# pranoyr/attention-models

Measured on AMD Instinct MI355X. Metric: ViTVQGAN 256px train-step images/sec, higher is better.
Workload: dtype f32; 1 GPU; BASELINE.json configs[2]: ViTVQGAN dim=256 patch=8 img=256 depth=6+6 h=8 d=64 mlp=2048 (SwiGLU), codebook 8192x32; GAN train step (D phase + G phase, gradient penalty, per_loss_weight=0), Adam, clip 1.0; global_batch=32, batch_per_gpu=32, parallelism=dp1

## Files before the change

attention-models_amd/amk/lib.py:

```python
import ctypes
import os
import re

_HERE = os.path.dirname(os.path.abspath(__file__))
LIB_PATH = os.environ.get("AMK_LIB") or os.path.join(_HERE, "libamk.so")
HEADER_PATH = os.path.normpath(os.path.join(_HERE, "..", "..", "include", "amk.h"))

AMK_OK = 0

_c = ctypes
_P = _c.c_void_p
_I = _c.c_int
_L = _c.c_int64
_F = _c.c_float



class GemmDesc(_c.Structure):
    _fields_ = [("op", _c.c_int32), ("epilogue", _c.c_int32), ("m", _L),
                ("n", _c.c_int32), ("k", _c.c_int32), ("split", _c.c_int32), ("reserved", _c.c_int32),
                ("a", _P), ("a2", _P), ("w", _P), ("w2", _P), ("c", _P), ("c2", _P),
                ("lda", _L), ("lda2", _L), ("ldw", _L), ("ldw2", _L), ("ldc", _L), ("ldc2", _L),
                ("bias", _P), ("bias2", _P), ("resid", _P), ("ldr", _L),
                ("ln_mean", _P), ("ln_rstd", _P), ("ln_gamma", _P), ("ln_beta", _P),
                ("ab", _P), ("ldab", _L), ("gate", _P), ("ldg", _L), ("dbias", _P)]


GEMM_NT, GEMM_NN, GEMM_TN = 0, 1, 2
EPI_BIAS, EPI_RESID, EPI_SWIGLU, EPI_SWIGLU_BWD = 0, 1, 2, 3

SIGNATURES = {
    "amk_version": (_I, []),
    "amk_arch": (_c.c_char_p, []),
    "amk_last_error": (_c.c_char_p, []),
    "amk_attn_fwd": (_I, [_P] * 7 + [_I] * 5 + [_L] * 12 + [_F, _P]),
    "amk_attn_scores_bytes": (_L, [_I, _I, _I, _I]),
    "amk_attn_fwd_keep": (_I, [_P] * 8 + [_I] * 5 + [_L] * 12 + [_F, _P]),
    "amk_attn_fwd_x6_ws_bytes": (_L, [_I, _I, _I]),
    "amk_attn_fwd_x6": (_I, [_P] * 8 + [_I] * 5 + [_L] * 12 + [_F, _P]),
    "amk_attn_bwd_ws_floats": (_L, [_I, _I, _I, _I, _I]),
    "amk_attn_bwd": (_I, [_P] * 12 + [_I] * 5 + [_L] * 24 + [_F, _I, _P]),
    "amk_attn_bwd_kept": (_I, [_P] * 13 + [_I] * 5 + [_L] * 24 + [_F, _I, _P]),
    "amk_vq_num_partials": (_L, [_L]),
    "amk_vq_lookup_fwd": (_I, [_P, _P, _L, _I, _I, _I] + [_P] * 9 + [_P]),
    "amk_vq_lookup_bwd": (_I, [_P] * 7 + [_F, _L, _I, _I, _P, _P, _P]),
    "amk_vq_lookup_bwd_rows": (_I, [_P] * 7 + [_F, _L, _I, _I, _P, _P, _P]),
    "amk_vq_padded_codes": (_I, [_I, _I]),
    "amk_vq_gather": (_I, [_P, _P, _L, _I, _I, _P, _P, _P]),
    "amk_agent_num_chunks": (_I, [_I]),
    "amk_agent_ws_floats": (_L, [_I, _I, _I, _I, _I]),
    "amk_agent_num_chunks_dh": (_I, [_I, _I]),
    "amk_agent_ws_floats_dh": (_L, [_I, _I, _I, _I, _I, _I]),
    "amk_agent_attn_fwd": (_I, [_P] * 10 + [_I] * 5 + [_L] * 12 + [_F, _P]),
    "amk_agent_attn_bwd": (_I, [_P] * 14 + [_I] * 5 + [_L] * 21 + [_F, _P]),
    "amk_agent_conv_grad_reduce": (_I, [_P, _P, _L, _I, _P, _P, _P]),
    "amk_rowsum_num_partials": (_I, [_L]),
    "amk_add_layernorm_fwd": (_I, [_P, _P, _P, _P, _L, _I, _F, _P, _P, _P, _P, _P]),
    "amk_add_layernorm_bwd": (_I, [_P, _P, _P, _P, _P, _P, _L, _I, _P, _P, _P]),
    "amk_colsum": (_I, [_P, _L, _I, _P, _P]),
    "amk_swiglu_fwd": (_I, [_P, _L, _I, _P, _P]),
    "amk_swiglu_bwd": (_I, [_P, _P, _L, _I, _P, _P]),
    "amk_geglu_fwd": (_I, [_P, _L, _I, _P, _P]),
# ... 89 lines not shown
```

attention-models_amd/amk/ops.py:

```python
import ctypes
import os
import weakref

import torch
from torch.autograd.function import once_differentiable

from . import lib as _lib

_NULL = ctypes.c_void_p(0)


def _ptr(t):
    return ctypes.c_void_p(t.data_ptr()) if t is not None else _NULL


def _stream():
    return ctypes.c_void_p(torch.cuda.current_stream().cuda_stream)


KERNEL_EVENTS = None


class _timed:

# ... 49 lines not shown
def _as_kernel_view(t):
    if _kernel_view_ok(t):
        return t
    B, H, T, D = t.shape
    return t.permute(0, 2, 1, 3).contiguous().permute(0, 2, 1, 3)


def _new_bthd(B, H, T, D, like):
    return torch.empty((B, T, H, D), device=like.device, dtype=torch.float32).permute(0, 2, 1, 3)


def _mask_u8(mask, shape, what):
    if mask is None:
        return None
    m = mask
    while m.dim() > len(shape) and m.shape[0] == 1:
        m = m[0]
    if m.dim() != len(shape):
        raise RuntimeError(f"{what} must have {len(shape)} dims (got shape {tuple(mask.shape)})")
    m = m.expand(*shape)
    return m.to(torch.uint8).contiguous()


ATTENTION_FORWARD = os.environ.get("AMK_ATTENTION_FORWARD", "f32")

ATTENTION_KEEP_SCORES = os.environ.get("AMK_ATTN_KEEP_SCORES", "1") == "1"
ATTENTION_KEEP_SCORES_MAX_BYTES = 8 << 30
ATTENTION_KEEP_SCORES_BUDGET_BYTES = int(os.environ.get("AMK_ATTN_KEEP_BUDGET", "0")) or None
_kept_scores_bytes = [0]


def _keep_budget(device):
    if ATTENTION_KEEP_SCORES_BUDGET_BYTES is not None:
        return ATTENTION_KEEP_SCORES_BUDGET_BYTES
    return torch.cuda.get_device_properties(device).total_memory // 4


def _release_kept(nbytes):
    _kept_scores_bytes[0] -= nbytes
ATTENTION_BACKWARD_KEYS = int(os.environ.get("AMK_ATTN_BWD_KEYS", "0"))


def _attn_forward(q, k, v, key_mask, causal_mask, scale, keep_scores=False):
    B, H, I, D = q.shape
    J = k.shape[2]
    _require_device(q, k, v, key_mask, causal_mask)
    if k.shape != (B, H, J, D) or v.shape != (B, H, J, D):
        raise RuntimeError(f"attention shapes disagree: q {tuple(q.shape)} k {tuple(k.shape)} v {tuple(v.shape)}")
    q, k, v = _as_kernel_view(q), _as_kernel_view(k), _as_kernel_view(v)
    o = _new_bthd(B, H, I, D, q)
    stats = torch.empty((B, H, I, 2), device=q.device, dtype=torch.float32)
    L = _lib.load()
    x6 = ATTENTION_FORWARD == "bf16x6" and D == 64
    ws = torch.empty((L.amk_attn_fwd_x6_ws_bytes(B, H, J),), device=q.device, dtype=torch.uint8) if x6 else None
    scores = None
    det = DETERMINISTIC_ATTENTION_BACKWARD or torch.are_deterministic_algorithms_enabled()
    keepable = D == 64 or (D == 128 and key_mask is None and causal_mask is None and not det)
    if (keep_scores and keepable and not x6 and ATTENTION_KEEP_SCORES
            and not ATTENTION_BACKWARD_TWO_KERNEL):
        nbytes = L.amk_attn_scores_bytes(B, H, I, J)
        if nbytes <= ATTENTION_KEEP_SCORES_MAX_BYTES and _kept_scores_bytes[0] + nbytes <= _keep_budget(q.device):
            scores = torch.empty((nbytes // 4,), device=q.device, dtype=torch.float32)
            _kept_scores_bytes[0] += nbytes
            weakref.finalize(scores.untyped_storage(), _release_kept, nbytes)
    with _timed("attn_fwd_keep_kernel" if scores is not None else "attn_fwd_kernel"):
        if scores is not None:
            rc = L.amk_attn_fwd_keep(
                _ptr(q), _ptr(k), _ptr(v), _ptr(o), _ptr(stats), _ptr(scores), _ptr(key_mask), _ptr(causal_mask),
                B, H, I, J, D, *_strides4(q), *_strides4(k), *_strides4(v), *_strides4(o),
                float(scale), _stream(),
            )
        elif x6:
            rc = L.amk_attn_fwd_x6(
                _ptr(q), _ptr(k), _ptr(v), _ptr(o), _ptr(stats), _ptr(ws), _ptr(key_mask), _ptr(causal_mask),
                B, H, I, J, D, *_strides4(q), *_strides4(k), *_strides4(v), *_strides4(o),
                float(scale), _stream(),
            )
        else:
            rc = L.amk_attn_fwd(
                _ptr(q), _ptr(k), _ptr(v), _ptr(o), _ptr(stats), _ptr(key_mask), _ptr(causal_mask),
                B, H, I, J, D, *_strides4(q), *_strides4(k), *_strides4(v), *_strides4(o),
                float(scale), _stream(),
            )
    _lib.check(rc, "amk_attn_fwd")
    return q, k, v, o, stats, scores


DETERMINISTIC_ATTENTION_BACKWARD = os.environ.get("AMK_DETERMINISTIC", "0") == "1"
ATTENTION_BACKWARD_TWO_KERNEL = False
# ... 42 lines not shown
        )
        _lib.check(rc, "amk_attn_bwd")

    if KERNEL_EVENTS is not None and (stages & ATTN_BWD_DELTA) and (stages & ~ATTN_BWD_DELTA):
        call(ATTN_BWD_DELTA)
        name = "attn_bwd_dkdv+dq" if not stages & ATTN_BWD_FUSED else (
            "attn_bwd_fused_kernel(kept scores)" if scores is not None else "attn_bwd_fused_kernel")
        with _timed(name):
            call(stages & ~ATTN_BWD_DELTA)
    else:
        call(stages)


_amp_fwd = torch.amp.custom_fwd(device_type="cuda", cast_inputs=torch.float32)
_amp_bwd = torch.amp.custom_bwd(device_type="cuda")


class _AttnCore(torch.autograd.Function):

    @staticmethod
    @_amp_fwd
    def forward(ctx, q, k, v, key_mask, causal_mask, scale):
        need = any(ctx.needs_input_grad[:3])
        q, k, v, o, stats, scores = _attn_forward(q, k, v, key_mask, causal_mask, scale, keep_scores=need)
        ctx.save_for_backward(q, k, v, o, stats, key_mask, causal_mask, scores)
        ctx.scale = scale
        return o

    @staticmethod
    @once_differentiable
    @_amp_bwd
    def backward(ctx, d_o):
        q, k, v, o, stats, key_mask, causal_mask, scores = ctx.saved_tensors
        B, H, I, D = q.shape
        J = k.shape[2]
        dq = _new_bthd(B, H, I, D, q)
        dk = _new_bthd(B, H, J, D, q)
        dv = _new_bthd(B, H, J, D, q)
        _attn_backward(q, k, v, o, stats, d_o, dq, dk, dv, key_mask, causal_mask, ctx.scale, scores=scores)
        return dq, dk, dv, None, None, None


class _AttnFusedKV(torch.autograd.Function):

    @staticmethod
    @_amp_fwd
    def forward(ctx, q2, kv2, key_mask, causal_mask, H, D, scale):
        B, I, _ = q2.shape
        J = kv2.shape[1]
        q2 = q2.contiguous()
        kv2 = kv2.contiguous()
        q = q2.view(B, I, H, D).permute(0, 2, 1, 3)
        kv = kv2.view(B, J, 2, H, D)
        k = kv[:, :, 0].permute(0, 2, 1, 3)
        v = kv[:, :, 1].permute(0, 2, 1, 3)
        need = any(ctx.needs_input_grad[:2])
        q, k, v, o, stats, scores = _attn_forward(q, k, v, key_mask, causal_mask, scale, keep_scores=need)
        ctx.save_for_backward(q, k, v, o, stats, key_mask, causal_mask, scores)
        ctx.scale = scale
        return o.permute(0, 2, 1, 3).reshape(B, I, H * D)

    @staticmethod
    @once_differentiable
    @_amp_bwd
    def backward(ctx, d_o2):
        q, k, v, o, stats, key_mask, causal_mask, scores = ctx.saved_tensors
        B, H, I, D = q.shape
        J = k.shape[2]
        d_o = d_o2.contiguous().view(B, I, H, D).permute(0, 2, 1, 3)
        dq2 = torch.empty((B, I, H * D), device=q.device, dtype=torch.float32)
        dkv2 = torch.empty((B, J, 2 * H * D), device=q.device, dtype=torch.float32)
        dq = dq2.view(B, I, H, D).permute(0, 2, 1, 3)
        dkv = dkv2.view(B, J, 2, H, D)
        dk = dkv[:, :, 0].permute(0, 2, 1, 3)
        dv = dkv[:, :, 1].permute(0, 2, 1, 3)
        _attn_backward(q, k, v, o, stats, d_o, dq, dk, dv, key_mask, causal_mask, ctx.scale, scores=scores)
        return dq2, dkv2, None, None, None, None, None


ATTENTION_BF16 = os.environ.get("AMK_ATTENTION_BF16", "1") == "1"
# ... 1502 lines not shown
```

attention-models_amd/csrc/attn_common.h:

```cpp
#pragma once
#include "amk_common.h"

namespace amk_attn {

constexpr int D = 64;
constexpr int NWAVE = 4;
constexpr int WG = NWAVE * AMK_WAVE;
constexpr int BLK = 32 * NWAVE;
constexpr int TILE = 64;
constexpr int LDS_STRIDE = 68;

#define AMK_FILL_MASKED (-1.0e9f * AMK_LOG2E)

struct Strides {
  int64_t sb, st, sh;
};

struct FwdParams {
  const float *q, *k, *v;
  float *o, *stats;
  const uint8_t *key_mask, *causal_mask;
  int B, H, I, J;
  Strides qs, ks, vs, os;
  float scale;
// ... 51 lines not shown
#pragma unroll
    for (int ps = 0; ps < NP; ++ps) {
      dst[ps] = __builtin_bit_cast(float4, __builtin_amdgcn_raw_buffer_load_b128(rsrc, voff[ps], 0, 0));
      voff[ps] += step;
    }
  }
  __device__ __forceinline__ void seek(int blk, int64_t row_stride, int tid) {
    const int srow = tid >> 4, scol = (tid & 15) * 4;
#pragma unroll
    for (int ps = 0; ps < NP; ++ps) voff[ps] = (int)(((int64_t)(srow + RP * ps) * row_stride + scol) * 4) + blk * step;
  }
};
typedef RowStagerT<TILE> RowStager;

inline bool aligned16(const void* p) { return (reinterpret_cast<uintptr_t>(p) & 15) == 0; }
inline bool strides_ok(const Strides& s) { return (s.sb % 4 == 0) && (s.st % 4 == 0) && (s.sh % 4 == 0); }

__device__ __forceinline__ float4 ld4(const float* p) { return *reinterpret_cast<const float4*>(p); }
__device__ __forceinline__ void st4(float* p, float4 v) { *reinterpret_cast<float4*>(p) = v; }
__device__ __forceinline__ float f4(const float4& v, int e) {
  return e == 0 ? v.x : (e == 1 ? v.y : (e == 2 ? v.z : v.w));
}

void launch_attn_fwd_x6(const FwdParams& p, int64_t nwg, hipStream_t st);

bool launch_attn_bwd_fused(const BwdParams& p, int keys_per_wg, hipStream_t st);
int fused_keys_per_wg(int J, int keys_per_wg);

bool attn_gen_supported(int Dh);
void launch_attn_fwd_gen(const FwdParams& p, int Dh, int64_t nwg, hipStream_t st);
void launch_attn_bwd_gen(const BwdParams& p, int Dh, int stages, hipStream_t st);
bool launch_attn_bwd_fused_gen(const BwdParams& p, int Dh, hipStream_t st);

}
```

attention-models_amd/csrc/attn_fwd.hip:

```cpp
#include "attn_common.h"
#include <stdlib.h>
#include <type_traits>

#ifndef AMK_FWD_ABL
#define AMK_FWD_ABL 0
#endif

namespace amk_attn {

template <bool CAUSAL, bool SCHED, bool KEEP>
__global__ __launch_bounds__(WG, 2) void attn_fwd_kernel(FwdParams p) {
  __shared__ __attribute__((aligned(16))) float smem[2 * TILE * LDS_STRIDE + TILE];
  float* Ks = smem;
  float* Vs = smem + TILE * LDS_STRIDE;
  float* Kfill = smem + 2 * TILE * LDS_STRIDE;

  const int tid = threadIdx.x;
  const int lane = tid & 63, wave = tid >> 6;
  const int ln = lane & 31, hf = lane >> 5;

  const int wg = __builtin_amdgcn_readfirstlane(xcd_remap(blockIdx.x, gridDim.x));
  const int qb = __builtin_amdgcn_readfirstlane(wg % p.nblk);
  const int bh = __builtin_amdgcn_readfirstlane(wg / p.nblk);
  const int h = __builtin_amdgcn_readfirstlane(bh % p.H), b = __builtin_amdgcn_readfirstlane(bh / p.H);
// ... 457 lines not shown
  FwdParams p;
  p.q = q; p.k = k; p.v = v; p.o = o; p.stats = stats;
  p.key_mask = key_mask; p.causal_mask = causal_mask;
  p.B = B; p.H = H; p.I = I; p.J = J;
  p.qs = {q_sb, q_st, q_sh}; p.ks = {k_sb, k_st, k_sh}; p.vs = {v_sb, v_st, v_sh}; p.os = {o_sb, o_st, o_sh};
  p.scale = scale;
  p.pinf = INFINITY;
  p.nblk = (I + BLK - 1) / BLK;
  p.x6_ws = x6_ws;
  p.scores = scores;
  AMK_CHECK_ARG(!scores || aligned16(scores), "amk_attn_fwd_keep: the scores buffer must be 16-byte aligned");
  AMK_CHECK_ARG(!x6 || (x6_ws && aligned16(x6_ws)), "amk_attn_fwd_x6: workspace missing or not 16-byte aligned");
  AMK_CHECK_ARG(aligned16(q) && aligned16(k) && aligned16(v) && aligned16(o) && strides_ok(p.qs) &&
                    strides_ok(p.ks) && strides_ok(p.vs) && strides_ok(p.os),
                "amk_attn_fwd: pointers must be 16-byte aligned and strides multiples of 4 elements");
  const int64_t nwg = (int64_t)B * H * p.nblk;
  AMK_CHECK_SUPPORTED(nwg < (1ll << 31), "amk_attn_fwd: grid too large");
  AMK_CHECK_SUPPORTED(((int64_t)J + TILE) * k_st * 4 < (1ll << 31) && ((int64_t)J + TILE) * v_st * 4 < (1ll << 31),
                      "amk_attn_fwd: one (batch, head) K/V slab must span < 2 GiB");
  hipStream_t st = static_cast<hipStream_t>(stream);
  if (Dh != D)
    launch_attn_fwd_gen(p, Dh, nwg, st);
  else if (x6)
    launch_attn_fwd_x6(p, nwg, st);
  else if (!causal_mask && !key_mask && getenv_plain() && scores)
    hipLaunchKernelGGL((attn_fwd_plain_kernel<true>), dim3((unsigned)nwg), dim3(WG), 0, st, p);
  else if (!causal_mask && !key_mask && getenv_plain())
    hipLaunchKernelGGL((attn_fwd_plain_kernel<false>), dim3((unsigned)nwg), dim3(WG), 0, st, p);
  else if (causal_mask && scores)
    hipLaunchKernelGGL((attn_fwd_kernel<true, false, true>), dim3((unsigned)nwg), dim3(WG), 0, st, p);
  else if (causal_mask)
    hipLaunchKernelGGL((attn_fwd_kernel<true, false, false>), dim3((unsigned)nwg), dim3(WG), 0, st, p);
  else if (scores)
    hipLaunchKernelGGL((attn_fwd_kernel<false, true, true>), dim3((unsigned)nwg), dim3(WG), 0, st, p);
  else
    hipLaunchKernelGGL((attn_fwd_kernel<false, true, false>), dim3((unsigned)nwg), dim3(WG), 0, st, p);
  AMK_CHECK_LAUNCH("amk_attn_fwd");
  return AMK_OK;
}

extern "C" int amk_attn_fwd(const float* q, const float* k, const float* v, float* o, float* stats,
                            const uint8_t* key_mask, const uint8_t* causal_mask,
                            int B, int H, int I, int J, int Dh,
                            int64_t q_sb, int64_t q_st, int64_t q_sh,
                            int64_t k_sb, int64_t k_st, int64_t k_sh,
                            int64_t v_sb, int64_t v_st, int64_t v_sh,
                            int64_t o_sb, int64_t o_st, int64_t o_sh,
// ... 16 lines not shown
                                 int64_t o_sb, int64_t o_st, int64_t o_sh,
                                 float scale, void* stream) {
  AMK_CHECK_ARG(scores, "amk_attn_fwd_keep: null scores buffer");
  return attn_fwd_impl(nullptr, false, scores, q, k, v, o, stats, key_mask, causal_mask, B, H, I, J, Dh, q_sb, q_st, q_sh, k_sb,
                       k_st, k_sh, v_sb, v_st, v_sh, o_sb, o_st, o_sh, scale, stream);
}

extern "C" int64_t amk_attn_fwd_x6_ws_bytes(int B, int H, int J) {
  if (B <= 0 || H <= 0 || J <= 0) return 0;
  return (int64_t)B * H * ((J + TILE - 1) / TILE) * 2 * 24576;
}

extern "C" int amk_attn_fwd_x6(const float* q, const float* k, const float* v, float* o, float* stats, void* ws,
                               const uint8_t* key_mask, const uint8_t* causal_mask,
                               int B, int H, int I, int J, int Dh,
                               int64_t q_sb, int64_t q_st, int64_t q_sh,
                               int64_t k_sb, int64_t k_st, int64_t k_sh,
                               int64_t v_sb, int64_t v_st, int64_t v_sh,
                               int64_t o_sb, int64_t o_st, int64_t o_sh,
                               float scale, void* stream) {
  return attn_fwd_impl(ws, true, nullptr, q, k, v, o, stats, key_mask, causal_mask, B, H, I, J, Dh, q_sb, q_st, q_sh, k_sb, k_st, k_sh,
                       v_sb, v_st, v_sh, o_sb, o_st, o_sh, scale, stream);
}
```

attention-models_amd/csrc/attn_fwd_x6.hip:

```cpp
#include "attn_common.h"

namespace amk_attn {

typedef __bf16 bf16x8 __attribute__((ext_vector_type(8)));
typedef __bf16 bf16x4 __attribute__((ext_vector_type(4)));

constexpr int PSTR = 72;
constexpr int PLANE = TILE * PSTR;

__device__ __forceinline__ f32x16 mfmab(bf16x8 a, bf16x8 b, f32x16 c) {
  return __builtin_amdgcn_mfma_f32_32x32x16_bf16(a, b, c, 0, 0, 0);
}
__device__ __forceinline__ f32x16 mfma6(const bf16x8 (&a)[3], const bf16x8 (&b)[3], f32x16 c) {
  c = mfmab(a[1], b[1], c);
  c = mfmab(a[2], b[0], c);
  c = mfmab(a[0], b[2], c);
  c = mfmab(a[1], b[0], c);
  c = mfmab(a[0], b[1], c);
  c = mfmab(a[0], b[0], c);
  return c;
}
__device__ __forceinline__ void mfma6x2(const bf16x8 (&a0)[3], const bf16x8 (&a1)[3], const bf16x8 (&b)[3], f32x16& c0, f32x16& c1) {
  c0 = mfmab(a0[1], b[1], c0); c1 = mfmab(a1[1], b[1], c1);
  c0 = mfmab(a0[2], b[0], c0); c1 = mfmab(a1[2], b[0], c1);
// ... 6 lines not shown
  h = (__bf16)x;
  const float r1 = x - (float)h;
  m = (__bf16)r1;
  l = (__bf16)(r1 - (float)m);
}
__device__ __forceinline__ void split8(const float (&x)[8], bf16x8 (&pl)[3]) {
#pragma unroll
  for (int j = 0; j < 8; ++j) {
    __bf16 h, m, l;
    split1(x[j], h, m, l);
    pl[0][j] = h; pl[1][j] = m; pl[2][j] = l;
  }
}
__device__ __forceinline__ void split4(float a, float b, float c, float d, bf16x4 (&pl)[3]) {
  const float x[4] = {a, b, c, d};
#pragma unroll
  for (int j = 0; j < 4; ++j) {
    __bf16 h, m, l;
    split1(x[j], h, m, l);
    pl[0][j] = h; pl[1][j] = m; pl[2][j] = l;
  }
}

template <bool CAUSAL>
__global__ __launch_bounds__(WG, 2) void attn_fwd_x6_kernel(FwdParams p) {
  __shared__ __attribute__((aligned(16))) __bf16 Kp[3 * PLANE];
  __shared__ __attribute__((aligned(16))) __bf16 Vt[3 * PLANE];
  __shared__ __attribute__((aligned(16))) float Kfill[TILE];

  const int tid = threadIdx.x;
  const int lane = tid & 63, wave = tid >> 6;
  const int ln = lane & 31, hf = lane >> 5;

  const int wg = xcd_remap(blockIdx.x, gridDim.x);
  const int qb = wg % p.nblk;
  const int bh = wg / p.nblk;
  const int h = bh % p.H, b = bh / p.H;

  const int qi = qb * BLK + wave * 32 + ln;
  const bool qvalid = qi < p.I;

  bf16x8 qpl[4][3];
  {
    const float qscale = p.scale * AMK_LOG2E;
    const float* qp = p.q + (int64_t)b * p.qs.sb + (int64_t)qi * p.qs.st + (int64_t)h * p.qs.sh + 8 * hf;
#pragma unroll
    for (int c = 0; c < 4; ++c) {
      const float4 t0 = qvalid ? ld4(qp + 16 * c) : make_float4(0.f, 0.f, 0.f, 0.f);
      const float4 t1 = qvalid ? ld4(qp + 16 * c + 4) : make_float4(0.f, 0.f, 0.f, 0.f);
      const float x[8] = {t0.x * qscale, t0.y * qscale, t0.z * qscale, t0.w * qscale,
                          t1.x * qscale, t1.y * qscale, t1.z * qscale, t1.w * qscale};
      split8(x, qpl[c]);
    }
  }

  const uint8_t* kmask = p.key_mask ? p.key_mask + (int64_t)b * p.J : nullptr;
  const uint8_t* cmrow = CAUSAL ? p.causal_mask + (int64_t)qi * p.J : nullptr;

  const int ntile = (p.J + TILE - 1) / TILE;
  const __amdgpu_buffer_rsrc_t wsrc = __builtin_amdgcn_make_buffer_rsrc(
      reinterpret_cast<char*>(p.x6_ws) + (int64_t)bh * ntile * 2 * 24576, 0, ntile * 2 * 24576, 0x00020000);
  float4 kch[6], vch[6];
  int lds_off[6];
#pragma unroll
  for (int n = 0; n < 6; ++n) {
    const int c = tid + 256 * n;
    const int row = c / 24, plane = (c % 24) >> 3, k8 = c & 7;
    lds_off[n] = plane * PLANE + row * PSTR + 8 * k8;
  }
  float fillst = 0.f;
  auto prefetch = [&](int t) {
    const int base = t * 2 * 24576 + tid * 16;
#pragma unroll
    for (int n = 0; n < 6; ++n) {
      kch[n] = __builtin_bit_cast(float4, __builtin_amdgcn_raw_buffer_load_b128(wsrc, base + 4096 * n, 0, 0));
      vch[n] = __builtin_bit_cast(float4, __builtin_amdgcn_raw_buffer_load_b128(wsrc, base + 24576 + 4096 * n, 0, 0));
    }
    if (tid < TILE) {
      const int j = t * TILE + tid;
      float f = 0.f;
      if (j >= p.J) f = -INFINITY;
      else if (kmask && kmask[j] == 0) f = AMK_FILL_MASKED;
      fillst = f;
    }
  };
  auto commit = [&]() {
#pragma unroll
    for (int n = 0; n < 6; ++n) {
      *reinterpret_cast<float4*>(&Kp[lds_off[n]]) = kch[n];
      *reinterpret_cast<float4*>(&Vt[lds_off[n]]) = vch[n];
    }
    if (tid < TILE) Kfill[tid] = fillst;
  };

  f32x16 o0 = zero16(), o1 = zero16();
  float m_run = -INFINITY, l_run = 0.f;

  prefetch(0);
  for (int t = 0; t < ntile; ++t) {
    const int j0 = t * TILE;
    __syncthreads();
    commit();
    __syncthreads();
    if (t + 1 < ntile) prefetch(t + 1);

    unsigned cbits0 = 0, cbits1 = 0;
    if (CAUSAL) {
      if (qvalid) {
#pragma unroll
        for (int r = 0; r < 16; ++r) {
          const int ja = j0 + acc_row(r, hf), jb = ja + 32;
          if (ja < p.J && cmrow[ja]) cbits0 |= 1u << r;
          if (jb < p.J && cmrow[jb]) cbits1 |= 1u << r;
        }
      }
    }

    f32x16 s0 = zero16(), s1 = zero16();
#pragma unroll
    for (int c = 0; c < 4; ++c) {
      bf16x8 ka[3], kb2[3];
#pragma unroll
      for (int q = 0; q < 3; ++q) {
        ka[q] = *reinterpret_cast<const bf16x8*>(&Kp[q * PLANE + ln * PSTR + 16 * c + 8 * hf]);
        kb2[q] = *reinterpret_cast<const bf16x8*>(&Kp[q * PLANE + (32 + ln) * PSTR + 16 * c + 8 * hf]);
      }
      mfma6x2(ka, kb2, qpl[c], s0, s1);
    }

    const bool plain = !CAUSAL && kmask == nullptr && (j0 + TILE <= p.J);
    float mx;
    if (plain) {
      mx = vmax(s0[0], s1[0], p.pinf);
#pragma unroll
      for (int r = 1; r < 16; ++r) mx = vmax(mx, vmax(s0[r], s1[r], p.pinf), p.pinf);
    } else {
      mx = -INFINITY;
#pragma unroll
      for (int g = 0; g < 4; ++g) {
        const float4 f0 = ld4(&Kfill[8 * g + 4 * hf]);
        const float4 f1 = ld4(&Kfill[32 + 8 * g + 4 * hf]);
#pragma unroll
        for (int e = 0; e < 4; ++e) {
          const int r = 4 * g + e;
          float t0 = s0[r], t1 = s1[r];
          const float fa = f4(f0, e), fb = f4(f1, e);
          t0 = (fa == 0.f) ? t0 : fa;
          t1 = (fb == 0.f) ? t1 : fb;
          if (CAUSAL) {
            t0 = ((cbits0 >> r) & 1u) ? AMK_FILL_MASKED : t0;
            t1 = ((cbits1 >> r) & 1u) ? AMK_FILL_MASKED : t1;
// ... 8 lines not shown
    const float m_new = vmax(m_run, mx, p.pinf);
    f32x2 lsum2 = {0.f, 0.f};
#pragma unroll
    for (int r = 0; r < 16; ++r) {
      const float p0 = __builtin_amdgcn_exp2f(s0[r] - m_new);
      const float p1 = __builtin_amdgcn_exp2f(s1[r] - m_new);
      s0[r] = p0;
      s1[r] = p1;
      lsum2 += (f32x2){p0, p1};
    }
    const float lsum = lsum2.x + lsum2.y;
    if (__any(m_new != m_run)) {
      const float alpha = __builtin_amdgcn_exp2f(m_run - m_new);
      l_run *= alpha;
#pragma unroll
      for (int r = 0; r < 16; ++r) {
        o0[r] *= alpha;
        o1[r] *= alpha;
      }
      m_run = m_new;
    }
    l_run += lsum;

#pragma unroll
    for (int g = 0; g < 4; ++g) {
      float x[8];
#pragma unroll
      for (int j = 0; j < 8; ++j) x[j] = (g < 2) ? s0[8 * (g & 1) + j] : s1[8 * (g & 1) + j];
      bf16x8 pp[3];
      split8(x, pp);
      bf16x8 va[3], vb[3];
#pragma unroll
      for (int q = 0; q < 3; ++q) {
        va[q] = *reinterpret_cast<const bf16x8*>(&Vt[q * PLANE + ln * PSTR + 16 * g + 8 * hf]);
        vb[q] = *reinterpret_cast<const bf16x8*>(&Vt[q * PLANE + (32 + ln) * PSTR + 16 * g + 8 * hf]);
      }
      mfma6x2(va, vb, pp, o0, o1);
    }
  }

  const float l_tot = l_run + __shfl_xor(l_run, 32, 64);
  const float inv = 1.f / l_tot;
  if (qvalid) {
    float* op = p.o + (int64_t)b * p.os.sb + (int64_t)qi * p.os.st + (int64_t)h * p.os.sh + 4 * hf;
#pragma unroll
    for (int g = 0; g < 4; ++g) {
      st4(op + 8 * g, make_float4(o0[4 * g] * inv, o0[4 * g + 1] * inv, o0[4 * g + 2] * inv, o0[4 * g + 3] * inv));
      st4(op + 32 + 8 * g, make_float4(o1[4 * g] * inv, o1[4 * g + 1] * inv, o1[4 * g + 2] * inv, o1[4 * g + 3] * inv));
    }
    if (hf == 0) {
      float* sp = p.stats + (((int64_t)b * p.H + h) * p.I + qi) * 2;
      sp[0] = m_run;
      sp[1] = l_tot;
    }
  }
}

__global__ __launch_bounds__(WG) void attn_split_kv_kernel(FwdParams p) {
  const int tid = threadIdx.x;
  const int ntile = (p.J + TILE - 1) / TILE;
  const int t = blockIdx.x % ntile;
  const int bh = blockIdx.x / ntile;
  const int h = bh % p.H, b = bh / p.H;
  const float* kbase = p.k + (int64_t)b * p.ks.sb + (int64_t)h * p.ks.sh;
  const float* vbase = p.v + (int64_t)b * p.vs.sb + (int64_t)h * p.vs.sh;
  __bf16* out = reinterpret_cast<__bf16*>(p.x6_ws) + ((int64_t)bh * ntile + t) * 2 * 1536 * 8;
  const int srow = tid >> 4, scol = (tid & 15) * 4;
  RowStager kload, vload;
  kload.init(kbase, p.ks.st, p.J, tid);
  vload.init(vbase, p.vs.st, p.J, tid);
  kload.seek(t, p.ks.st, tid);
  vload.seek(t, p.vs.st, tid);
#pragma unroll
  for (int i = 0; i < 4; ++i) vload.voff[i] = (int)(((int64_t)(4 * srow + i) * p.vs.st + scol) * 4) + t * vload.step;
  float4 kst[4], vst[4];
  kload.load(kst);
  vload.load(vst);
#pragma unroll
  for (int ps = 0; ps < 4; ++ps) {
    bf16x4 pl[3];
    split4(kst[ps].x, kst[ps].y, kst[ps].z, kst[ps].w, pl);
    const int r = srow + 16 * ps;
#pragma unroll
    for (int q = 0; q < 3; ++q) *reinterpret_cast<bf16x4*>(out + (r * 3 + q) * 64 + scol) = pl[q];
  }
  const int vpos = 16 * (srow >> 2) + 4 * (((srow & 1) << 1) | ((srow >> 1) & 1));
  __bf16* vout = out + 1536 * 8;
#pragma unroll
  for (int dd = 0; dd < 4; ++dd) {
    bf16x4 pl[3];
    split4(f4(vst[0], dd), f4(vst[1], dd), f4(vst[2], dd), f4(vst[3], dd), pl);
#pragma unroll
    for (int q = 0; q < 3; ++q) *reinterpret_cast<bf16x4*>(vout + ((scol + dd) * 3 + q) * 64 + vpos) = pl[q];
  }
}

void launch_attn_fwd_x6(const FwdParams& p, int64_t nwg, hipStream_t st) {
  const int ntile = (p.J + TILE - 1) / TILE;
  hipLaunchKernelGGL(attn_split_kv_kernel, dim3((unsigned)((int64_t)p.B * p.H * ntile)), dim3(WG), 0, st, p);
  if (p.causal_mask)
    hipLaunchKernelGGL(attn_fwd_x6_kernel<true>, dim3((unsigned)nwg), dim3(WG), 0, st, p);
  else
    hipLaunchKernelGGL(attn_fwd_x6_kernel<false>, dim3((unsigned)nwg), dim3(WG), 0, st, p);
}

}
```

include/amk.h:

```cpp
#ifndef AMK_H_
#define AMK_H_

#include <stdint.h>

#ifdef __cplusplus
extern "C" {
#endif

#define AMK_VERSION 140

enum {
  AMK_OK = 0,
  AMK_EINVAL = -1,
  AMK_EUNSUPPORTED = -2,
  AMK_ELAUNCH = -3
};

int amk_version(void);
const char* amk_arch(void);
const char* amk_last_error(void);

int amk_attn_fwd(const float* q, const float* k, const float* v, float* o, float* stats,
                 const uint8_t* key_mask, const uint8_t* causal_mask,
                 int B, int H, int I, int J, int D,
// ... 2 lines not shown
                 int64_t v_sb, int64_t v_st, int64_t v_sh,
                 int64_t o_sb, int64_t o_st, int64_t o_sh,
                 float scale, void* stream);

int64_t amk_attn_scores_bytes(int B, int H, int I, int J);
int amk_attn_fwd_keep(const float* q, const float* k, const float* v, float* o, float* stats, float* scores,
                      const uint8_t* key_mask, const uint8_t* causal_mask,
                      int B, int H, int I, int J, int D,
                      int64_t q_sb, int64_t q_st, int64_t q_sh,
                      int64_t k_sb, int64_t k_st, int64_t k_sh,
                      int64_t v_sb, int64_t v_st, int64_t v_sh,
                      int64_t o_sb, int64_t o_st, int64_t o_sh,
                      float scale, void* stream);

int64_t amk_attn_fwd_x6_ws_bytes(int B, int H, int J);
int amk_attn_fwd_x6(const float* q, const float* k, const float* v, float* o, float* stats, void* ws,
                    const uint8_t* key_mask, const uint8_t* causal_mask,
                    int B, int H, int I, int J, int D,
                    int64_t q_sb, int64_t q_st, int64_t q_sh,
                    int64_t k_sb, int64_t k_st, int64_t k_sh,
                    int64_t v_sb, int64_t v_st, int64_t v_sh,
                    int64_t o_sb, int64_t o_st, int64_t o_sh,
                    float scale, void* stream);

#define AMK_ATTN_BWD_DELTA 1
#define AMK_ATTN_BWD_DKDV 2
#define AMK_ATTN_BWD_DQ 4
#define AMK_ATTN_BWD_FUSED 8
#define AMK_ATTN_BWD_ALL 7
#define AMK_ATTN_BWD_FAST 9
#define AMK_ATTN_BWD_KEYS128 16
#define AMK_ATTN_BWD_KEYS256 32
#define AMK_ATTN_BWD_DQ_REPRO 64
#define AMK_ATTN_BWD_FAST_REPRO 73
int64_t amk_attn_bwd_ws_floats(int B, int H, int I, int J, int stages);
int amk_attn_bwd(const float* q, const float* k, const float* v, const float* o,
                 const float* stats, const float* d_o,
                 float* dq, float* dk, float* dv, float* delta_ws,
                 const uint8_t* key_mask, const uint8_t* causal_mask,
                 int B, int H, int I, int J, int D,
                 int64_t q_sb, int64_t q_st, int64_t q_sh,
                 int64_t k_sb, int64_t k_st, int64_t k_sh,
                 int64_t v_sb, int64_t v_st, int64_t v_sh,
                 int64_t o_sb, int64_t o_st, int64_t o_sh,
                 int64_t do_sb, int64_t do_st, int64_t do_sh,
                 int64_t dq_sb, int64_t dq_st, int64_t dq_sh,
// ... 245 lines not shown
```

Measured before the change: 307.7 images/s.

## Enable bf16x6 attention forward by default with score-keeping and lazy-rescale plain kernel

Switches the attention forward default from f32 to an auto mode that uses the split-bf16 (x6) MFMA kernel when head dim is 64 and the problem is large enough. Adds a keep-scores variant of the x6 kernel so backward can reuse stored scores, plus a plain (no-mask) x6 kernel with lazy max rescaling (threshold tau) and buffer-resource loads. It also marks wave-uniform indices with readfirstlane. The aim is to replace slower f32 FMA attention with matrix-core work, at the cost of more kernel variants and possible small numerical differences.

New measurement: 312.9 images/s, median of 6. +1.7%, better.

```diff
diff --git a/attention-models_amd/amk/lib.py b/attention-models_amd/amk/lib.py
--- a/attention-models_amd/amk/lib.py
+++ b/attention-models_amd/amk/lib.py
@@ -38,6 +38,7 @@
     "amk_attn_fwd_keep": (_I, [_P] * 8 + [_I] * 5 + [_L] * 12 + [_F, _P]),
     "amk_attn_fwd_x6_ws_bytes": (_L, [_I, _I, _I]),
     "amk_attn_fwd_x6": (_I, [_P] * 8 + [_I] * 5 + [_L] * 12 + [_F, _P]),
+    "amk_attn_fwd_x6_keep": (_I, [_P] * 9 + [_I] * 5 + [_L] * 12 + [_F, _P]),
     "amk_attn_bwd_ws_floats": (_L, [_I, _I, _I, _I, _I]),
     "amk_attn_bwd": (_I, [_P] * 12 + [_I] * 5 + [_L] * 24 + [_F, _I, _P]),
     "amk_attn_bwd_kept": (_I, [_P] * 13 + [_I] * 5 + [_L] * 24 + [_F, _I, _P]),
diff --git a/attention-models_amd/amk/ops.py b/attention-models_amd/amk/ops.py
--- a/attention-models_amd/amk/ops.py
+++ b/attention-models_amd/amk/ops.py
@@ -95,7 +95,11 @@
     return m.to(torch.uint8).contiguous()
 
 
-ATTENTION_FORWARD = os.environ.get("AMK_ATTENTION_FORWARD", "f32")
+ATTENTION_FORWARD = os.environ.get("AMK_ATTENTION_FORWARD", "auto")
+if ATTENTION_FORWARD not in ("auto", "f32", "bf16x6"):
+    raise RuntimeError(f"AMK_ATTENTION_FORWARD must be auto, f32 or bf16x6 (got {ATTENTION_FORWARD!r})")
+ATTENTION_X6_MIN_KEYS = 128
+ATTENTION_X6_MIN_SCORES = 1 << 22
 
 ATTENTION_KEEP_SCORES = os.environ.get("AMK_ATTN_KEEP_SCORES", "1") == "1"
 ATTENTION_KEEP_SCORES_MAX_BYTES = 8 << 30
@@ -114,7 +118,7 @@
 ATTENTION_BACKWARD_KEYS = int(os.environ.get("AMK_ATTN_BWD_KEYS", "0"))
 
 
-def _attn_forward(q, k, v, key_mask, causal_mask, scale, keep_scores=False):
+def _attn_forward(q, k, v, key_mask, causal_mask, scale, keep_scores=False, auto_x6=False):
     B, H, I, D = q.shape
     J = k.shape[2]
     _require_device(q, k, v, key_mask, causal_mask)
@@ -124,20 +128,29 @@
     o = _new_bthd(B, H, I, D, q)
     stats = torch.empty((B, H, I, 2), device=q.device, dtype=torch.float32)
     L = _lib.load()
-    x6 = ATTENTION_FORWARD == "bf16x6" and D == 64
+    if ATTENTION_FORWARD not in ("auto", "f32", "bf16x6"):
+        raise RuntimeError(f"ops.ATTENTION_FORWARD must be auto, f32 or bf16x6 (got {ATTENTION_FORWARD!r})")
+    x6 = D == 64 and (ATTENTION_FORWARD == "bf16x6"
+                      or (ATTENTION_FORWARD == "auto" and auto_x6 and J >= ATTENTION_X6_MIN_KEYS
+                          and B * H * I * J >= ATTENTION_X6_MIN_SCORES))
     ws = torch.empty((L.amk_attn_fwd_x6_ws_bytes(B, H, J),), device=q.device, dtype=torch.uint8) if x6 else None
     scores = None
     det = DETERMINISTIC_ATTENTION_BACKWARD or torch.are_deterministic_algorithms_enabled()
     keepable = D == 64 or (D == 128 and key_mask is None and causal_mask is None and not det)
-    if (keep_scores and keepable and not x6 and ATTENTION_KEEP_SCORES
-            and not ATTENTION_BACKWARD_TWO_KERNEL):
+    if keep_scores and keepable and ATTENTION_KEEP_SCORES and not ATTENTION_BACKWARD_TWO_KERNEL:
         nbytes = L.amk_attn_scores_bytes(B, H, I, J)
         if nbytes <= ATTENTION_KEEP_SCORES_MAX_BYTES and _kept_scores_bytes[0] + nbytes <= _keep_budget(q.device):
             scores = torch.empty((nbytes // 4,), device=q.device, dtype=torch.float32)
             _kept_scores_bytes[0] += nbytes
             weakref.finalize(scores.untyped_storage(), _release_kept, nbytes)
-    with _timed("attn_fwd_keep_kernel" if scores is not None else "attn_fwd_kernel"):
-        if scores is not None:
+    with _timed(("attn_fwd_x6" if x6 else "attn_fwd") + ("_keep_kernel" if scores is not None else "_kernel")):
+        if x6 and scores is not None:
+            rc = L.amk_attn_fwd_x6_keep(
+                _ptr(q), _ptr(k), _ptr(v), _ptr(o), _ptr(stats), _ptr(ws), _ptr(scores), _ptr(key_mask), _ptr(causal_mask),
+                B, H, I, J, D, *_strides4(q), *_strides4(k), *_strides4(v), *_strides4(o),
+                float(scale), _stream(),
+            )
+        elif scores is not None:
             rc = L.amk_attn_fwd_keep(
                 _ptr(q), _ptr(k), _ptr(v), _ptr(o), _ptr(stats), _ptr(scores), _ptr(key_mask), _ptr(causal_mask),
                 B, H, I, J, D, *_strides4(q), *_strides4(k), *_strides4(v), *_strides4(o),
@@ -226,7 +239,7 @@
     @_amp_fwd
     def forward(ctx, q, k, v, key_mask, causal_mask, scale):
         need = any(ctx.needs_input_grad[:3])
-        q, k, v, o, stats, scores = _attn_forward(q, k, v, key_mask, causal_mask, scale, keep_scores=need)
+        q, k, v, o, stats, scores = _attn_forward(q, k, v, key_mask, causal_mask, scale, keep_scores=need, auto_x6=True)
         ctx.save_for_backward(q, k, v, o, stats, key_mask, causal_mask, scores)
         ctx.scale = scale
         return o
@@ -259,7 +272,7 @@
         k = kv[:, :, 0].permute(0, 2, 1, 3)
         v = kv[:, :, 1].permute(0, 2, 1, 3)
         need = any(ctx.needs_input_grad[:2])
-        q, k, v, o, stats, scores = _attn_forward(q, k, v, key_mask, causal_mask, scale, keep_scores=need)
+        q, k, v, o, stats, scores = _attn_forward(q, k, v, key_mask, causal_mask, scale, keep_scores=need, auto_x6=True)
         ctx.save_for_backward(q, k, v, o, stats, key_mask, causal_mask, scores)
         ctx.scale = scale
         return o.permute(0, 2, 1, 3).reshape(B, I, H * D)
diff --git a/attention-models_amd/csrc/attn_common.h b/attention-models_amd/csrc/attn_common.h
--- a/attention-models_amd/csrc/attn_common.h
+++ b/attention-models_amd/csrc/attn_common.h
@@ -97,7 +97,7 @@
   return e == 0 ? v.x : (e == 1 ? v.y : (e == 2 ? v.z : v.w));
 }
 
-void launch_attn_fwd_x6(const FwdParams& p, int64_t nwg, hipStream_t st);
+void launch_attn_fwd_x6(const FwdParams& p, int64_t nwg, hipStream_t st, bool plain);
 
 bool launch_attn_bwd_fused(const BwdParams& p, int keys_per_wg, hipStream_t st);
 int fused_keys_per_wg(int J, int keys_per_wg);
diff --git a/attention-models_amd/csrc/attn_fwd.hip b/attention-models_amd/csrc/attn_fwd.hip
--- a/attention-models_amd/csrc/attn_fwd.hip
+++ b/attention-models_amd/csrc/attn_fwd.hip
@@ -503,7 +503,7 @@
   if (Dh != D)
     launch_attn_fwd_gen(p, Dh, nwg, st);
   else if (x6)
-    launch_attn_fwd_x6(p, nwg, st);
+    launch_attn_fwd_x6(p, nwg, st, getenv_plain());
   else if (!causal_mask && !key_mask && getenv_plain() && scores)
     hipLaunchKernelGGL((attn_fwd_plain_kernel<true>), dim3((unsigned)nwg), dim3(WG), 0, st, p);
   else if (!causal_mask && !key_mask && getenv_plain())
@@ -566,3 +566,16 @@
   return attn_fwd_impl(ws, true, nullptr, q, k, v, o, stats, key_mask, causal_mask, B, H, I, J, Dh, q_sb, q_st, q_sh, k_sb, k_st, k_sh,
                        v_sb, v_st, v_sh, o_sb, o_st, o_sh, scale, stream);
 }
+
+extern "C" int amk_attn_fwd_x6_keep(const float* q, const float* k, const float* v, float* o, float* stats, void* ws, float* scores,
+                                    const uint8_t* key_mask, const uint8_t* causal_mask,
+                                    int B, int H, int I, int J, int Dh,
+                                    int64_t q_sb, int64_t q_st, int64_t q_sh,
+                                    int64_t k_sb, int64_t k_st, int64_t k_sh,
+                                    int64_t v_sb, int64_t v_st, int64_t v_sh,
+                                    int64_t o_sb, int64_t o_st, int64_t o_sh,
+                                    float scale, void* stream) {
+  AMK_CHECK_ARG(scores, "amk_attn_fwd_x6_keep: null scores buffer");
+  return attn_fwd_impl(ws, true, scores, q, k, v, o, stats, key_mask, causal_mask, B, H, I, J, Dh, q_sb, q_st, q_sh, k_sb, k_st,
+                       k_sh, v_sb, v_st, v_sh, o_sb, o_st, o_sh, scale, stream);
+}
diff --git a/attention-models_amd/csrc/attn_fwd_x6.hip b/attention-models_amd/csrc/attn_fwd_x6.hip
--- a/attention-models_amd/csrc/attn_fwd_x6.hip
+++ b/attention-models_amd/csrc/attn_fwd_x6.hip
@@ -1,4 +1,5 @@
 #include "attn_common.h"
+#include <type_traits>
 
 namespace amk_attn {
 
@@ -52,7 +53,77 @@
   }
 }
 
-template <bool CAUSAL>
+
+__device__ __forceinline__ void load_q_planes(const FwdParams& p, int b, int h, int qi, int hf, bool qvalid, bf16x8 (&qpl)[4][3]) {
+  const float qscale = p.scale * AMK_LOG2E;
+  const float* qp = p.q + (int64_t)b * p.qs.sb + (int64_t)qi * p.qs.st + (int64_t)h * p.qs.sh + 8 * hf;
+#pragma unroll
+  for (int c = 0; c < 4; ++c) {
+    const float4 t0 = qvalid ? ld4(qp + 16 * c) : make_float4(0.f, 0.f, 0.f, 0.f);
+    const float4 t1 = qvalid ? ld4(qp + 16 * c + 4) : make_float4(0.f, 0.f, 0.f, 0.f);
+    const float x[8] = {t0.x * qscale, t0.y * qscale, t0.z * qscale, t0.w * qscale,
+                        t1.x * qscale, t1.y * qscale, t1.z * qscale, t1.w * qscale};
+    split8(x, qpl[c]);
+  }
+}
+__device__ __forceinline__ void st_x6(const __bf16* Kp, const bf16x8 (&qpl)[4][3], int ln, int hf, f32x16& s0, f32x16& s1) {
+#pragma unroll
+  for (int c = 0; c < 4; ++c) {
+    bf16x8 ka[3], kb2[3];
+#pragma unroll
+    for (int q = 0; q < 3; ++q) {
+      ka[q] = *reinterpret_cast<const bf16x8*>(&Kp[q * PLANE + ln * PSTR + 16 * c + 8 * hf]);
+      kb2[q] = *reinterpret_cast<const bf16x8*>(&Kp[q * PLANE + (32 + ln) * PSTR + 16 * c + 8 * hf]);
+    }
+    mfma6x2(ka, kb2, qpl[c], s0, s1);
+  }
+}
+__device__ __forceinline__ void pv_x6(const __bf16* Vt, const f32x16& s0, const f32x16& s1, int ln, int hf, f32x16& o0, f32x16& o1) {
+#pragma unroll
+  for (int g = 0; g < 4; ++g) {
+    float x[8];
+#pragma unroll
+    for (int j = 0; j < 8; ++j) x[j] = (g < 2) ? s0[8 * (g & 1) + j] : s1[8 * (g & 1) + j];
+    bf16x8 pp[3];
+    split8(x, pp);
+    bf16x8 va[3], vb[3];
+#pragma unroll
+    for (int q = 0; q < 3; ++q) {
+      va[q] = *reinterpret_cast<const bf16x8*>(&Vt[q * PLANE + ln * PSTR + 16 * g + 8 * hf]);
+      vb[q] = *reinterpret_cast<const bf16x8*>(&Vt[q * PLANE + (32 + ln) * PSTR + 16 * g + 8 * hf]);
+    }
+    mfma6x2(va, vb, pp, o0, o1);
+  }
+}
+__device__ __forceinline__ void keep_x6(float* sc_ptr, int64_t sc_kstep, int t, const f32x16& s0, const f32x16& s1) {
+  float* t0 = sc_ptr + (int64_t)(2 * t) * sc_kstep;
+  float* t1 = t0 + sc_kstep;
+#pragma unroll
+  for (int r = 0; r < 16; ++r) {
+    __builtin_nontemporal_store(s0[r], t0 + acc_row(r, 0) * 32);
+    __builtin_nontemporal_store(s1[r], t1 + acc_row(r, 0) * 32);
+  }
+}
+__device__ __forceinline__ void epilogue_x6(const FwdParams& p, int b, int h, int qi, int hf, bool qvalid, const f32x16& o0,
+                                            const f32x16& o1, float m_ref, float l_run) {
+  const float l_tot = l_run + __shfl_xor(l_run, 32, 64);
+  const float inv = 1.f / l_tot;
+  if (qvalid) {
+    float* op = p.o + (int64_t)b * p.os.sb + (int64_t)qi * p.os.st + (int64_t)h * p.os.sh + 4 * hf;
+#pragma unroll
+    for (int g = 0; g < 4; ++g) {
+      st4(op + 8 * g, make_float4(o0[4 * g] * inv, o0[4 * g + 1] * inv, o0[4 * g + 2] * inv, o0[4 * g + 3] * inv));
+      st4(op + 32 + 8 * g, make_float4(o1[4 * g] * inv, o1[4 * g + 1] * inv, o1[4 * g + 2] * inv, o1[4 * g + 3] * inv));
+    }
+    if (hf == 0) {
+      float* sp = p.stats + (((int64_t)b * p.H + h) * p.I + qi) * 2;
+      sp[0] = m_ref;
+      sp[1] = l_tot;
+    }
+  }
+}
+
+template <bool CAUSAL, bool KEEP>
 __global__ __launch_bounds__(WG, 2) void attn_fwd_x6_kernel(FwdParams p) {
   __shared__ __attribute__((aligned(16))) __bf16 Kp[3 * PLANE];
   __shared__ __attribute__((aligned(16))) __bf16 Vt[3 * PLANE];
@@ -62,27 +133,16 @@
   const int lane = tid & 63, wave = tid >> 6;
   const int ln = lane & 31, hf = lane >> 5;
 
-  const int wg = xcd_remap(blockIdx.x, gridDim.x);
-  const int qb = wg % p.nblk;
-  const int bh = wg / p.nblk;
-  const int h = bh % p.H, b = bh / p.H;
+  const int wg = __builtin_amdgcn_readfirstlane(xcd_remap(blockIdx.x, gridDim.x));
+  const int qb = __builtin_amdgcn_readfirstlane(wg % p.nblk);
+  const int bh = __builtin_amdgcn_readfirstlane(wg / p.nblk);
+  const int h = __builtin_amdgcn_readfirstlane(bh % p.H), b = __builtin_amdgcn_readfirstlane(bh / p.H);
 
   const int qi = qb * BLK + wave * 32 + ln;
   const bool qvalid = qi < p.I;
 
   bf16x8 qpl[4][3];
-  {
-    const float qscale = p.scale * AMK_LOG2E;
-    const float* qp = p.q + (int64_t)b * p.qs.sb + (int64_t)qi * p.qs.st + (int64_t)h * p.qs.sh + 8 * hf;
-#pragma unroll
-    for (int c = 0; c < 4; ++c) {
-      const float4 t0 = qvalid ? ld4(qp + 16 * c) : make_float4(0.f, 0.f, 0.f, 0.f);
-      const float4 t1 = qvalid ? ld4(qp + 16 * c + 4) : make_float4(0.f, 0.f, 0.f, 0.f);
-      const float x[8] = {t0.x * qscale, t0.y * qscale, t0.z * qscale, t0.w * qscale,
-                          t1.x * qscale, t1.y * qscale, t1.z * qscale, t1.w * qscale};
-      split8(x, qpl[c]);
-    }
-  }
+  load_q_planes(p, b, h, qi, hf, qvalid, qpl);
 
   const uint8_t* kmask = p.key_mask ? p.key_mask + (int64_t)b * p.J : nullptr;
   const uint8_t* cmrow = CAUSAL ? p.causal_mask + (int64_t)qi * p.J : nullptr;
@@ -125,6 +185,11 @@
 
   f32x16 o0 = zero16(), o1 = zero16();
   float m_run = -INFINITY, l_run = 0.f;
+
+  const ScoreTiles stl(p.I, p.J);
+  const int64_t sc_kstep = (int64_t)stl.nqt * 1024;
+  float* sc_ptr = nullptr;
+  if (KEEP) sc_ptr = p.scores + ((int64_t)bh * stl.nkb * stl.nqt + (qb * NWAVE + wave)) * 1024 + 4 * hf * 32 + ln;
 
   prefetch(0);
   for (int t = 0; t < ntile; ++t) {
@@ -147,16 +212,8 @@
     }
 
     f32x16 s0 = zero16(), s1 = zero16();
-#pragma unroll
-    for (int c = 0; c < 4; ++c) {
-      bf16x8 ka[3], kb2[3];
-#pragma unroll
-      for (int q = 0; q < 3; ++q) {
-        ka[q] = *reinterpret_cast<const bf16x8*>(&Kp[q * PLANE + ln * PSTR + 16 * c + 8 * hf]);
-        kb2[q] = *reinterpret_cast<const bf16x8*>(&Kp[q * PLANE + (32 + ln) * PSTR + 16 * c + 8 * hf]);
-      }
-      mfma6x2(ka, kb2, qpl[c], s0, s1);
-    }
+    st_x6(Kp, qpl, ln, hf, s0, s1);
+    if (KEEP) keep_x6(sc_ptr, sc_kstep, t, s0, s1);
 
     const bool plain = !CAUSAL && kmask == nullptr && (j0 + TILE <= p.J);
     float mx;
@@ -211,46 +268,139 @@
     }
     l_run += lsum;
 
-#pragma unroll
-    for (int g = 0; g < 4; ++g) {
-      float x[8];
-#pragma unroll
-      for (int j = 0; j < 8; ++j) x[j] = (g < 2) ? s0[8 * (g & 1) + j] : s1[8 * (g & 1) + j];
-      bf16x8 pp[3];
-      split8(x, pp);
-      bf16x8 va[3], vb[3];
-#pragma unroll
-      for (int q = 0; q < 3; ++q) {
-        va[q] = *reinterpret_cast<const bf16x8*>(&Vt[q * PLANE + ln * PSTR + 16 * g + 8 * hf]);
-        vb[q] = *reinterpret_cast<const bf16x8*>(&Vt[q * PLANE + (32 + ln) * PSTR + 16 * g + 8 * hf]);
+    pv_x6(Vt, s0, s1, ln, hf, o0, o1);
+  }
+  epilogue_x6(p, b, h, qi, hf, qvalid, o0, o1, m_run, l_run);
+}
+
+constexpr float LAZY_TAU = 8.f;
+
+__device__ __forceinline__ float max3(float a, float b, float c) { return __builtin_fmaxf(__builtin_fmaxf(a, b), c); }
+
+template <bool KEEP>
+__global__ __launch_bounds__(WG, 2) void attn_fwd_x6_plain_kernel(FwdParams p) {
+  __shared__ __attribute__((aligned(16))) __bf16 Kp[3 * PLANE];
+  __shared__ __attribute__((aligned(16))) __bf16 Vt[3 * PLANE];
+
+  const int tid = threadIdx.x;
+  const int lane = tid & 63, wave = tid >> 6;
+  const int ln = lane & 31, hf = lane >> 5;
+
+  const int wg = __builtin_amdgcn_readfirstlane(xcd_remap(blockIdx.x, gridDim.x));
+  const int qb = __builtin_amdgcn_readfirstlane(wg % p.nblk);
+  const int bh = __builtin_amdgcn_readfirstlane(wg / p.nblk);
+  const int h = __builtin_amdgcn_readfirstlane(bh % p.H), b = __builtin_amdgcn_readfirstlane(bh / p.H);
+
+  const int qi = qb * BLK + wave * 32 + ln;
+  const bool qvalid = qi < p.I;
+
+  bf16x8 qpl[4][3];
+  load_q_planes(p, b, h, qi, hf, qvalid, qpl);
+
+  const int ntile = (p.J + TILE - 1) / TILE;
+  const int nfull = p.J / TILE;
+  const __amdgpu_buffer_rsrc_t wsrc = __builtin_amdgcn_make_buffer_rsrc(
+      reinterpret_cast<char*>(p.x6_ws) + (int64_t)bh * ntile * 2 * 24576, 0, ntile * 2 * 24576, 0x00020000);
+  float4 kch[6], vch[6];
+  int lds_off[6];
+#pragma unroll
+  for (int n = 0; n < 6; ++n) {
+    const int c = tid + 256 * n;
+    const int row = c / 24, plane = (c % 24) >> 3, k8 = c & 7;
+    lds_off[n] = plane * PLANE + row * PSTR + 8 * k8;
+  }
+  auto prefetch = [&](int t) {
+    const int base = t * 2 * 24576 + tid * 16;
+#pragma unroll
+    for (int n = 0; n < 6; ++n) {
+      kch[n] = __builtin_bit_cast(float4, __builtin_amdgcn_raw_buffer_load_b128(wsrc, base + 4096 * n, 0, 0));
+      vch[n] = __builtin_bit_cast(float4, __builtin_amdgcn_raw_buffer_load_b128(wsrc, base + 24576 + 4096 * n, 0, 0));
+    }
+  };
+  auto commit = [&]() {
+#pragma unroll
+    for (int n = 0; n < 6; ++n) {
+      *reinterpret_cast<float4*>(&Kp[lds_off[n]]) = kch[n];
+      *reinterpret_cast<float4*>(&Vt[lds_off[n]]) = vch[n];
+    }
+  };
+
+  f32x16 o0 = zero16(), o1 = zero16();
+  float mref = 0.f, l_run = 0.f;
+
+  const ScoreTiles stl(p.I, p.J);
+  const int64_t sc_kstep = (int64_t)stl.nqt * 1024;
+  float* sc_ptr = nullptr;
+  if (KEEP) sc_ptr = p.scores + ((int64_t)bh * stl.nkb * stl.nqt + (qb * NWAVE + wave)) * 1024 + 4 * hf * 32 + ln;
+
+  auto tile = [&](const int t, auto ragged_c) {
+    constexpr bool RAGGED = decltype(ragged_c)::value;
+    __syncthreads();
+    commit();
+    __syncthreads();
+    if (t + 1 < ntile) prefetch(t + 1);
+
+    f32x16 s0 = zero16(), s1 = zero16();
+    st_x6(Kp, qpl, ln, hf, s0, s1);
+    if (KEEP) keep_x6(sc_ptr, sc_kstep, t, s0, s1);
+    if (RAGGED) {
+      const int j0 = t * TILE;
+#pragma unroll
+      for (int r = 0; r < 16; ++r) {
+        s0[r] = (j0 + acc_row(r, hf) < p.J) ? s0[r] : -INFINITY;
+        s1[r] = (j0 + 32 + acc_row(r, hf) < p.J) ? s1[r] : -INFINITY;
       }
-      mfma6x2(va, vb, pp, o0, o1);
-    }
-  }
-
-  const float l_tot = l_run + __shfl_xor(l_run, 32, 64);
-  const float inv = 1.f / l_tot;
-  if (qvalid) {
-    float* op = p.o + (int64_t)b * p.os.sb + (int64_t)qi * p.os.st + (int64_t)h * p.os.sh + 4 * hf;
-#pragma unroll
-    for (int g = 0; g < 4; ++g) {
-      st4(op + 8 * g, make_float4(o0[4 * g] * inv, o0[4 * g + 1] * inv, o0[4 * g + 2] * inv, o0[4 * g + 3] * inv));
-      st4(op + 32 + 8 * g, make_float4(o1[4 * g] * inv, o1[4 * g + 1] * inv, o1[4 * g + 2] * inv, o1[4 * g + 3] * inv));
-    }
-    if (hf == 0) {
-      float* sp = p.stats + (((int64_t)b * p.H + h) * p.I + qi) * 2;
-      sp[0] = m_run;
-      sp[1] = l_tot;
-    }
-  }
+    }
+    float mx = max3(s0[0], s1[0], s0[1]);
+    mx = max3(mx, s1[1], s0[2]);
+#pragma unroll
+    for (int r = 2; r < 15; ++r) mx = max3(mx, s1[r], s0[r + 1]);
+    mx = __builtin_fmaxf(mx, s1[15]);
+    mx = __builtin_fmaxf(mx, __shfl_xor(mx, 32, 64));
+    mx -= mref;
+    if (t == 0 || __any(mx > LAZY_TAU)) {
+      const float d = t == 0 ? mx : __builtin_fmaxf(mx, 0.f);
+      if (t != 0) {
+        const float alpha = __builtin_amdgcn_exp2f(-d);
+        l_run *= alpha;
+#pragma unroll
+        for (int r = 0; r < 16; ++r) {
+          o0[r] *= alpha;
+          o1[r] *= alpha;
+        }
+      }
+      mref += d;
+    }
+#pragma unroll
+    for (int r = 0; r < 16; ++r) {
+      s0[r] = __builtin_amdgcn_exp2f(s0[r] - mref);
+      s1[r] = __builtin_amdgcn_exp2f(s1[r] - mref);
+    }
+    f32x2 lsa = {0.f, 0.f}, lsb = {0.f, 0.f};
+#pragma unroll
+    for (int r = 0; r < 16; r += 2) {
+      lsa += (f32x2){s0[r], s0[r + 1]};
+      lsb += (f32x2){s1[r], s1[r + 1]};
+    }
+    lsa += lsb;
+    l_run += lsa.x + lsa.y;
+
+    pv_x6(Vt, s0, s1, ln, hf, o0, o1);
+  };
+
+  prefetch(0);
+  for (int t = 0; t < nfull; ++t) tile(t, std::false_type{});
+  if (nfull < ntile) tile(nfull, std::true_type{});
+
+  epilogue_x6(p, b, h, qi, hf, qvalid, o0, o1, mref, l_run);
 }
 
 __global__ __launch_bounds__(WG) void attn_split_kv_kernel(FwdParams p) {
   const int tid = threadIdx.x;
   const int ntile = (p.J + TILE - 1) / TILE;
-  const int t = blockIdx.x % ntile;
-  const int bh = blockIdx.x / ntile;
-  const int h = bh % p.H, b = bh / p.H;
+  const int t = __builtin_amdgcn_readfirstlane(blockIdx.x % ntile);
+  const int bh = __builtin_amdgcn_readfirstlane(blockIdx.x / ntile);
+  const int h = __builtin_amdgcn_readfirstlane(bh % p.H), b = __builtin_amdgcn_readfirstlane(bh / p.H);
   const float* kbase = p.k + (int64_t)b * p.ks.sb + (int64_t)h * p.ks.sh;
   const float* vbase = p.v + (int64_t)b * p.vs.sb + (int64_t)h * p.vs.sh;
   __bf16* out = reinterpret_cast<__bf16*>(p.x6_ws) + ((int64_t)bh * ntile + t) * 2 * 1536 * 8;
@@ -284,13 +434,22 @@
   }
 }
 
-void launch_attn_fwd_x6(const FwdParams& p, int64_t nwg, hipStream_t st) {
+void launch_attn_fwd_x6(const FwdParams& p, int64_t nwg, hipStream_t st, bool plain) {
   const int ntile = (p.J + TILE - 1) / TILE;
-  hipLaunchKernelGGL(attn_split_kv_kernel, dim3((unsigned)((int64_t)p.B * p.H * ntile)), dim3(WG), 0, st, p);
-  if (p.causal_mask)
-    hipLaunchKernelGGL(attn_fwd_x6_kernel<true>, dim3((unsigned)nwg), dim3(WG), 0, st, p);
-  else
-    hipLaunchKernelGGL(attn_fwd_x6_kernel<false>, dim3((unsigned)nwg), dim3(WG), 0, st, p);
-}
-
-}
+  const dim3 grid((unsigned)nwg), block(WG);
+  hipLaunchKernelGGL(attn_split_kv_kernel, dim3((unsigned)((int64_t)p.B * p.H * ntile)), block, 0, st, p);
+  const bool keep = p.scores != nullptr;
+  if (p.causal_mask) {
+    if (keep) hipLaunchKernelGGL((attn_fwd_x6_kernel<true, true>), grid, block, 0, st, p);
+    else hipLaunchKernelGGL((attn_fwd_x6_kernel<true, false>), grid, block, 0, st, p);
+  } else if (p.key_mask || !plain) {
+    if (keep) hipLaunchKernelGGL((attn_fwd_x6_kernel<false, true>), grid, block, 0, st, p);
+    else hipLaunchKernelGGL((attn_fwd_x6_kernel<false, false>), grid, block, 0, st, p);
+  } else if (keep) {
+    hipLaunchKernelGGL((attn_fwd_x6_plain_kernel<true>), grid, block, 0, st, p);
+  } else {
+    hipLaunchKernelGGL((attn_fwd_x6_plain_kernel<false>), grid, block, 0, st, p);
+  }
+}
+
+}
diff --git a/include/amk.h b/include/amk.h
--- a/include/amk.h
+++ b/include/amk.h
@@ -48,6 +48,14 @@
                     int64_t v_sb, int64_t v_st, int64_t v_sh,
                     int64_t o_sb, int64_t o_st, int64_t o_sh,
                     float scale, void* stream);
+int amk_attn_fwd_x6_keep(const float* q, const float* k, const float* v, float* o, float* stats, void* ws, float* scores,
+                         const uint8_t* key_mask, const uint8_t* causal_mask,
+                         int B, int H, int I, int J, int D,
+                         int64_t q_sb, int64_t q_st, int64_t q_sh,
+                         int64_t k_sb, int64_t k_st, int64_t k_sh,
+                         int64_t v_sb, int64_t v_st, int64_t v_sh,
+                         int64_t o_sb, int64_t o_st, int64_t o_sh,
+                         float scale, void* stream);
 
 #define AMK_ATTN_BWD_DELTA 1
 #define AMK_ATTN_BWD_DKDV 2
```
